# dkohlsdorf/audio_pattern_discovery

Hardware: AMD Instinct MI355X
Metric: DTW cell-updates/sec (whole node) (higher is better)
Workload: dtype f32

## Files before the change

audio_pattern_discovery_amd/csrc/apd_internal.h:

```cpp
#pragma once
#include <hip/hip_runtime.h>
#include <stdint.h>

#include <iterator>
#include <map>
#include <set>
#include <string>
#include <type_traits>
#include <utility>
#include <vector>

#include "../../include/apd.h"

struct apd_context;
namespace apd {

constexpr int kTile = 16;
constexpr int kSlotsPerTile = kTile * kTile;
constexpr int kWave = 64;

struct BandSpec {
    float pct;
    uint32_t explicit_band;
    int use_explicit;
    float ins, del, mat;
};

struct AlignLaunch {
    const float *d_frames;
    uint32_t frames_bytes;
    const uint32_t *d_seq_off;
    const float *d_seq_nmax;
    const uint4 *d_tiles;
    uint32_t n_tiles;
    uint32_t n_seq;
    uint32_t dim, dpad;
    BandSpec band;
    float *d_slab;
    const uint32_t *d_nonfinite;
    uint32_t w_max;
    uint32_t n_max;
    int variant;
    int hybrid;
    int strict;
    float tau;
};

constexpr int kKernelDims[] = {8, 10, 13, 16, 20, 26};
constexpr bool is_kernel_dim(uint32_t d) { for (int k : kKernelDims) if ((uint32_t)k == d) return true; return false; }
constexpr uint32_t kernel_dim(uint32_t d) { for (int k : kKernelDims) if ((uint32_t)k >= d) return (uint32_t)k; return d; }
constexpr int max_cells_per_lane(uint32_t d) { return d <= 13 ? 9 : (d <= 16 ? 7 : 5); }
constexpr int max_strip_columns(uint32_t d) { return d <= 10 ? 13 : (d <= 13 ? 11 : max_cells_per_lane(d)); }

struct KernelGeom {
    enum Family : uint8_t { Generic, Systolic, Wide, Strip, BandedStrip, SharedColumns };
    Family family = Generic;
    uint8_t lanes_or_waves = 0;
    uint8_t cells = 0;

    constexpr int encode() const
    {
        constexpr int base[] = {0, 0, 10000, 20000, 30000, 40000};
        return family == Generic ? 0 : base[family] + lanes_or_waves * 100 + cells;
    }
    static constexpr KernelGeom decode(int key)
    {
        const Family f = key >= 100 && key < 10000 ? Systolic : key >= 10000 && key < 20000 ? Wide
                       : key >= 20000 && key < 30000 ? Strip : key >= 30000 && key < 40000 ? BandedStrip
                       : key >= 40000 && key < 50000 ? SharedColumns : Generic;
        if (f == Generic) return KernelGeom{};
        return KernelGeom{f, (uint8_t)((key % 10000) / 100), (uint8_t)(key % 100)};
    }
    constexpr uint32_t lanes_per_pair() const
    {
        return family == Systolic || family == SharedColumns ? lanes_or_waves : family == Wide ? 64u * lanes_or_waves : 64u;
    }
    constexpr uint32_t capacity() const { return (family == Wide ? 64u : 1u) * lanes_or_waves * cells; }
    constexpr bool operator==(KernelGeom o) const { return family == o.family && lanes_or_waves == o.lanes_or_waves && cells == o.cells; }
    constexpr bool operator<(KernelGeom o) const { return encode() < o.encode(); }
};

#define APD_SYSTOLIC_GEOMS(X) X(8, 5) X(8, 7) X(8, 9) X(16, 2) X(16, 3) X(16, 5) X(16, 7) X(16, 9) X(32, 5) X(32, 7) X(32, 9) \
                              X(64, 3) X(64, 5) X(64, 7) X(64, 9)
#define APD_WIDE_GEOMS(X) X(2, 5) X(2, 7) X(2, 9) X(4, 5) X(4, 7) X(4, 9) X(8, 5) X(8, 7) X(8, 9)
#define APD_STRIP_GEOMS(X) X(1, 3) X(1, 5) X(1, 7) X(1, 9) X(1, 11) X(1, 13) X(2, 3) X(2, 5) X(2, 7) X(2, 9) X(2, 11) X(2, 13) \
                           X(4, 3) X(4, 5) X(4, 7) X(4, 9) X(4, 11) X(4, 13)
#define APD_BANDED_STRIP_GEOMS(X) X(1, 5) X(1, 9) X(4, 5) X(4, 9)
#define APD_SHARED_COLUMN_GEOMS(X) X(16, 9)

#define APD_SYSTOLIC_ENTRY_(A, B) KernelGeom{KernelGeom::Systolic, A, B},
#define APD_WIDE_ENTRY_(A, B) KernelGeom{KernelGeom::Wide, A, B},
#define APD_STRIP_ENTRY_(A, B) KernelGeom{KernelGeom::Strip, A, B},
#define APD_BANDED_STRIP_ENTRY_(A, B) KernelGeom{KernelGeom::BandedStrip, A, B},
#define APD_SHARED_COLUMN_ENTRY_(A, B) KernelGeom{KernelGeom::SharedColumns, A, B},
constexpr KernelGeom kSystolicGeoms[] = {APD_SYSTOLIC_GEOMS(APD_SYSTOLIC_ENTRY_)};
constexpr KernelGeom kWideGeoms[] = {APD_WIDE_GEOMS(APD_WIDE_ENTRY_)};
constexpr KernelGeom kStripGeoms[] = {APD_STRIP_GEOMS(APD_STRIP_ENTRY_)};
constexpr KernelGeom kBandedStripGeoms[] = {APD_BANDED_STRIP_GEOMS(APD_BANDED_STRIP_ENTRY_)};
constexpr KernelGeom kSharedColumnGeoms[] = {APD_SHARED_COLUMN_GEOMS(APD_SHARED_COLUMN_ENTRY_)};
#undef APD_SYSTOLIC_ENTRY_
#undef APD_WIDE_ENTRY_
#undef APD_STRIP_ENTRY_
#undef APD_BANDED_STRIP_ENTRY_
#undef APD_SHARED_COLUMN_ENTRY_

template <class F, size_t... I>
bool with_kernel_dim_(uint32_t dim, F &&f, std::index_sequence<I...>)
{
    return ((dim == (uint32_t)kKernelDims[I] ? (f(std::integral_constant<int, kKernelDims[I]>{}), true) : false) || ...);
}
template <class F>
bool with_kernel_dim(uint32_t dim, F &&f) { return with_kernel_dim_(dim, f, std::make_index_sequence<std::size(kKernelDims)>{}); }

constexpr bool geom_instantiated(KernelGeom g, uint32_t dim)
{
    if (g.family == KernelGeom::Generic) return true;
    if (!is_kernel_dim(dim)) return false;
    const bool strip = g.family == KernelGeom::Strip;
    if (g.cells > (strip ? max_strip_columns(dim) : max_cells_per_lane(dim))) return false;
    auto on = [g](const auto &list) { for (KernelGeom e : list) if (e == g) return true; return false; };
    return g.family == KernelGeom::Systolic ? on(kSystolicGeoms) : g.family == KernelGeom::Wide ? on(kWideGeoms)
         : g.family == KernelGeom::SharedColumns ? on(kSharedColumnGeoms) : strip ? on(kStripGeoms) : on(kBandedStripGeoms);
}
template <size_t N>
constexpr bool geoms_round_trip(const KernelGeom (&list)[N])
{
    for (KernelGeom g : list) if (!(KernelGeom::decode(g.encode()) == g)) return false;
    return true;
}
static_assert(geoms_round_trip(kSystolicGeoms) && geoms_round_trip(kWideGeoms) && geoms_round_trip(kStripGeoms) &&
                  geoms_round_trip(kBandedStripGeoms) && geoms_round_trip(kSharedColumnGeoms), "a listed geometry has no integer code of its own");

__host__ __device__ constexpr int sweep_result_offset(int rows, int cols, int w) { return (cols - 1) - (rows - 1) + w; }
__host__ __device__ constexpr int sweep_capture_step(int rows, int cols, int w, int c)
{
    return (rows - 1) + sweep_result_offset(rows, cols, w) / c;
}
__host__ __device__ constexpr int sweep_steps_needed(int rows, int cols, int w, int c) { return sweep_capture_step(rows, cols, w, c) + 1; }
static_assert(sweep_result_offset(1000, 1024, 66) == 90 && sweep_capture_step(1000, 1024, 66, 9) == 1009 &&
                  sweep_steps_needed(1000, 1024, 66, 9) == 1010, "cfg 3's shape, rows the shorter sequence: lane 10 ends the sweep");
static_assert(sweep_steps_needed(1024, 1000, 66, 9) == 1028, "the same pair with the longer sequence as rows: u* = 42, lane 4");
static_assert(sweep_capture_step(40, 72, 34, 9) == 39 + 7 && (2 * 34 + 1 + 8) / 9 == 8,
              "|n - m| = w - 2: u* = 2w - 2 sits in the last active lane, nothing is cut at the end");
static_assert(sweep_steps_needed(2, 2, 2, 2) == 3 && sweep_steps_needed(72, 40, 34, 9) == 72, "smallest pair; u* = 2: lane 0");

constexpr int shared_column_unroll(int c) { return (c + 1) % 2 == 0 ? c + 1 : 2 * (c + 1); }
constexpr int shared_column_ring_min(int g, int c) { return (g - 1) * (c - 1) + 1 + 2 * shared_column_unroll(c); }
constexpr int shared_column_ring_frames(int g, int c) { return (shared_column_ring_min(g, c) + 16 + 7) / 8 * 8; }
constexpr uint32_t shared_column_slack(KernelGeom g)
{
    return (uint32_t)(shared_column_ring_frames(g.lanes_or_waves, g.cells) - shared_column_ring_min(g.lanes_or_waves, g.cells));
}
inline uint32_t host_w(const BandSpec &b, uint32_t n, uint32_t m);
inline bool shared_columns_qualify(const std::vector<uint32_t> &lens, uint32_t tile_a, uint32_t tile_b, const BandSpec &band,
                                   uint32_t slack)
{
    const uint32_t n_seq = (uint32_t)lens.size();
    for (uint32_t sa = 0; sa < (uint32_t)kTile; sa += 4)
        for (uint32_t sb = 0; sb < (uint32_t)kTile; sb += 4) {
            uint32_t lo = 0xFFFFFFFFu, hi = 0;
            for (uint32_t i = 0; i < 16; ++i) {
                const uint32_t a = tile_a * kTile + sa + i / 4, b = tile_b * kTile + sb + i % 4;
                if (!(a < b && b < n_seq) || lens[a] < 2 || lens[b] < 2) continue;
                const uint32_t w = host_w(band, lens[a], lens[b]);
                lo = w < lo ? w : lo;
                hi = w > hi ? w : hi;
            }
            if (hi > lo && hi - lo > slack) return false;
        }
    return true;
}

constexpr uint64_t strip_lds_bytes(uint32_t dim, uint32_t ppw, bool banded, uint32_t rows)
{
    const uint64_t dp = (dim + 4) & ~3u;
    return 4 * ((ppw == 1 ? 128 : 64) * dp + (uint64_t)ppw * (banded ? 2 : 1) * (rows + 4) + 16);
}

constexpr uint32_t kPathMaxOffsets = 20480;
__host__ __device__ constexpr uint32_t path_cells_per_lane(uint32_t w) { return (2 * w + 1 + 63) / 64 < 2 ? 2u : (2 * w + 1 + 63) / 64; }
inline uint64_t path_dir_words(uint32_t n, uint32_t m, uint32_t w)
{
    if (n < 2 || m < 2) return 0;
    return ((uint64_t)n + 63) * ((path_cells_per_lane(w) + 15) / 16) * 64;
}
struct PathPair {
    uint32_t px, py;
    uint64_t dir_off;
    uint64_t step_off;
};
struct PathLaunch {
    const float *d_frames;
    const uint32_t *d_seq_off;
    uint32_t dim, dpad;
    BandSpec band;
    const PathPair *d_pairs;
    uint32_t n_pairs;
    uint32_t *d_dirs;
    apd_path_step *d_steps;
    uint32_t *d_len;
    float *d_scores;
};
hipError_t launch_path_sweep(const PathLaunch &L, uint32_t c_max, hipStream_t stream);
hipError_t launch_path_trace(const PathLaunch &L, hipStream_t stream);

hipError_t launch_align(const AlignLaunch &L, KernelGeom g, hipStream_t stream, std::string &err, int *status);
hipError_t launch_generic_fallback(const AlignLaunch &L, hipStream_t stream, bool *fits);
bool generic_fallback_fits(uint32_t w_max);

struct TileClass { KernelGeom geom; uint32_t first, count, w_max, n_max; };
void plan_tile_classes(const std::vector<uint64_t> &offsets, uint32_t n_seq, const std::vector<uint2> &tiles, const BandSpec &band,
                       uint32_t dim, int variant, bool fast_ok, bool uniform_pen, bool fast_shift, std::vector<TileClass> &classes,
                       std::vector<uint4> &flat);
hipError_t launch_pad(const float *d_src, float *d_dst, const uint32_t *d_seq_off, const uint32_t *d_src_off, uint32_t n_seq,
                      uint64_t n_frames_padded, uint32_t src_dim, uint32_t dim, uint32_t dpad, uint32_t *d_flags, float *d_seq_nmax,
                      hipStream_t stream);
hipError_t launch_unpack(const float *d_gathered, float *d_out, const uint32_t *d_order, uint32_t n_seq, uint32_t world,
                         uint64_t slab_floats, const uint32_t *d_flags, uint32_t *d_status, hipStream_t stream);
hipError_t launch_selftest(int *d_result, hipStream_t stream);
hipError_t launch_join_flags(uint32_t *d_flags_out, const uint32_t *d_flags_a, const uint32_t *d_flags_b, hipStream_t stream);
hipError_t launch_unpack_cross(const float *d_slab, float *d_fs, float *d_sf, const uint32_t *d_order, uint32_t n_seq, uint32_t n0,
                               uint32_t n_first, bool swapped, const uint32_t *d_flags, uint32_t *d_status, hipStream_t stream);
hipError_t launch_cross_linkage(const float *d_fs, const float *d_sf, uint32_t n_first, uint32_t n_second, const uint32_t *d_members,
                                const uint32_t *d_set_off, uint32_t n_sets, float *d_link, uint32_t *d_nearest, float *d_nearest_linkage,
                                hipStream_t stream);
hipError_t launch_sqrt_sweep(uint32_t first, uint64_t count, unsigned long long *d_out, hipStream_t stream);
constexpr float kFeatureFloor = 0x1p-40f;
constexpr float kFeatureBound = 0x1p60f;

struct DeviceBuf {
    void *ptr = nullptr;
    size_t bytes = 0;
    DeviceBuf() = default;
    DeviceBuf(DeviceBuf &&o) noexcept : ptr(o.ptr), bytes(o.bytes) { o.ptr = nullptr; o.bytes = 0; }
    DeviceBuf &operator=(DeviceBuf &&o) noexcept { std::swap(ptr, o.ptr); std::swap(bytes, o.bytes); return *this; }
    ~DeviceBuf() { reset(); }
    hipError_t reset() { const hipError_t e = ptr ? hipFree(ptr) : hipSuccess; ptr = nullptr; bytes = 0; return e; }
    hipError_t alloc(size_t n)
    {
        if (hipError_t e = reset(); e != hipSuccess) return e;
        if (hipError_t e = hipMalloc(&ptr, n); e != hipSuccess) { ptr = nullptr; return e; }
        bytes = n;
        return hipSuccess;
    }
    hipError_t reserve(size_t n) { return ptr && bytes >= n ? hipSuccess : alloc(n); }
    template <class T> T *as() const { return static_cast<T *>(ptr); }
    explicit operator bool() const { return ptr != nullptr; }
};

struct ContextChild {
    apd_context *ctx = nullptr;
    virtual void release_device() = 0;
    virtual ~ContextChild() = default;
};
int destroy_child(ContextChild *child);

int device_select(apd_context *ctx, const float *d_x, uint64_t len, uint64_t k, float *value);
uint64_t percentile_index(uint64_t len, float perc);

inline uint32_t host_band_from_pct(float pct, uint32_t len)
{
    float p = pct * (float)len;
    if (!(p > 0.0f)) return 0;
    if (p >= 4294967040.0f) return 0xFFFFFFFFu;
    return (uint32_t)p;
}
inline uint32_t host_w(const BandSpec &b, uint32_t n, uint32_t m)
{
    uint32_t mx = n > m ? n : m, gap = n > m ? n - m : m - n;
    uint32_t band = b.use_explicit ? b.explicit_band : host_band_from_pct(b.pct, mx);
    if (band > mx) band = mx;
    return (band > gap ? band : gap) + 2;
}

extern thread_local const apd_context *tl_bound_context;
bool affinity_debug();
hipError_t bind_device(const apd_context *ctx);
bool affinity_ok(const apd_context *ctx, const char *where);

}

#define APD_AFFINITY(ctx, where)                                                                   \
    do { if (apd::affinity_debug() && !apd::affinity_ok((ctx), (where))) return APD_ERR_HIP; } while (0)

#define HIP_TRY(ctx, call)                                                             \
    do {                                                                               \
        if (hipError_t e_ = (call); e_ != hipSuccess) {                                \
            (ctx)->last_error = std::string(#call) + ": " + hipGetErrorString(e_);     \
            return e_ == hipErrorOutOfMemory ? APD_ERR_OOM : APD_ERR_HIP;              \
        }                                                                              \
    } while (0)

struct apd_context {
    int device = 0;
    hipStream_t stream = nullptr;
    bool own_stream = false;
    bool timing = false;
    hipEvent_t ev0 = nullptr, ev1 = nullptr;
    static constexpr int kSideStreams = 4;
    hipStream_t side[kSideStreams] = {nullptr, nullptr, nullptr, nullptr};
    hipEvent_t side_done[kSideStreams] = {nullptr, nullptr, nullptr, nullptr};
    hipEvent_t fork = nullptr;
    std::set<apd::ContextChild *> children;
    std::set<void *> buffers;
    bool timed = false;
    int variant = 0;
    int distance_mode = 1;
    float tau = 1.0f / 64.0f;
    std::string last_error;
    apd::DeviceBuf ws_linkage;
    apd::DeviceBuf ws_slab;
    apd::DeviceBuf ws_misc;
    apd::DeviceBuf ws_gather;
    apd::DeviceBuf ws_path_dirs;
    apd::DeviceBuf ws_path_steps;
    uint32_t *d_status = nullptr;
    uint32_t drop_tiles = 0;
    apd_batch *pair_batch = nullptr;
    uint64_t pair_n = 0, pair_m = 0;
    uint32_t pair_dim = 0;
};

inline int reserve_ws(apd_context *ctx, apd::DeviceBuf &ws, size_t need)
{
    APD_AFFINITY(ctx, "workspace allocation");
    HIP_TRY(ctx, ws.reserve(need));
    return APD_OK;
}

struct apd_batch : apd::ContextChild {
    uint32_t n_seq = 0, dim = 0, dpad = 0;
    uint32_t src_dim = 0;
    uint64_t total_frames = 0;
    apd::DeviceBuf d_frames;
    uint32_t frames_bytes = 0;
    apd::DeviceBuf d_meta;
    std::vector<uint32_t> h_meta;
    uint32_t *d_seq_off = nullptr;
    uint32_t *d_src_off = nullptr;
    uint32_t *d_order = nullptr;
    uint32_t *d_flags = nullptr;
    float *d_seq_nmax = nullptr;
    mutable int nonfinite = -1;
    std::vector<uint32_t> order;
    std::vector<uint64_t> offsets;
    uint32_t min_len = 0, max_len = 0;
    bool joined = false, swapped = false;
    uint32_t first_len = 0, seg0 = 0;
    struct TilePlan { apd::DeviceBuf d_tiles; std::vector<apd::TileClass> classes; };
    mutable std::map<std::string, TilePlan> tile_cache;
    void release_device() override;
};
```

audio_pattern_discovery_amd/csrc/dtw_systolic.h:

```cpp
#pragma once
#include <type_traits>

#ifndef APD_ABLATE
#define APD_ABLATE 0
#endif

#include "dtw_common.h"

namespace apd {

typedef float apd_f32x4 __attribute__((ext_vector_type(4)));
constexpr uint32_t kNoFrame = 0xFFFFFF00u;

template <int D>
__device__ __forceinline__ void load_frame(float (&dst)[D], __amdgpu_buffer_rsrc_t rsrc, uint32_t byte_off)
{
    constexpr int DP4 = (D + 3) / 4;
#pragma unroll
    for (int q = 0; q < DP4; ++q) {
        const apd_f32x4 t = __builtin_bit_cast(apd_f32x4, __builtin_amdgcn_raw_buffer_load_b128(rsrc, byte_off + 16u * q, 0, 0));
        if (4 * q + 0 < D) dst[4 * q + 0] = t.x;
        if (4 * q + 1 < D) dst[4 * q + 1] = t.y;
        if (4 * q + 2 < D) dst[4 * q + 2] = t.z;
        if (4 * q + 3 < D) dst[4 * q + 3] = t.w;
    }
}

template <int D>
__device__ __forceinline__ void load_frame_dwords(float (&dst)[D], __amdgpu_buffer_rsrc_t rsrc, uint32_t byte_off)
{
#pragma unroll
    for (int k = 0; k < D; ++k)
        dst[k] = __builtin_bit_cast(float, __builtin_amdgcn_raw_buffer_load_b32(rsrc, byte_off + 4u * k, 0, 0));
}

template <int D, int DN>
__device__ __forceinline__ float frame_dist(const float (&x)[DN], const float (&y)[DN])
{
    float t = x[0] - y[0];
    float acc = t * t;
#pragma unroll
    for (int k = 1; k < D; ++k) {
        t = x[k] - y[k];
        acc = __builtin_fmaf(t, t, acc);
    }
    if (APD_ABLATE & 1) return acc;
    return __builtin_amdgcn_sqrtf(acc);
}

template <int D, int DN>
__device__ __forceinline__ float frame_sq_strict(const float (&x)[DN], const float (&y)[DN])
{
    float t = x[0] - y[0];
    float acc = t * t;
#pragma unroll
    for (int k = 1; k < D; ++k) {
        t = x[k] - y[k];
        const float sq = t * t;
        acc = acc + sq;
    }
    return acc;
}
template <int D, int DN>
__device__ __forceinline__ float frame_dist_strict(const float (&x)[DN], const float (&y)[DN])
{
    return __builtin_sqrtf(frame_sq_strict<D, DN>(x, y));
}

template <int D>
__device__ __forceinline__ float frame_sq_expanded_pre(const float (&xm)[D + 1], const float (&y)[D + 1])
{
    float acc = xm[D] + y[D];
#pragma unroll
    for (int k = 0; k < D; ++k) acc = __builtin_fmaf(xm[k], y[k], acc);
    return acc;
}
template <int D>
__device__ __forceinline__ void prescale_row_piece(apd_f32x4 &v, int piece)
{
    const bool np = piece == D / 4;
    v.x = (np && D % 4 == 0) ? v.x : -2.0f * v.x;
    v.y = (np && D % 4 == 1) ? v.y : -2.0f * v.y;
    v.z = (np && D % 4 == 2) ? v.z : -2.0f * v.z;
    v.w = (np && D % 4 == 3) ? v.w : -2.0f * v.w;
}
template <int D>
__device__ __forceinline__ float frame_sq_exact_pre(const float (&xm)[D + 1], const float (&y)[D + 1])
{
    float t = __builtin_fmaf(-0.5f, xm[0], -y[0]);
    float acc = t * t;
#pragma unroll
    for (int k = 1; k < D; ++k) {
        t = __builtin_fmaf(-0.5f, xm[k], -y[k]);
        acc = __builtin_fmaf(t, t, acc);
    }
    return acc;
}
template <int C, int G, bool UNIFORM_PEN>
__device__ __forceinline__ void dp_rows_step(float (&prev1)[C], float (&prev2)[C], const float (&d)[C], const bool (&g1)[C],
                                             const bool (&g2)[C], float del, float ins, float mat, int gl)
{
    float left1 = group_from_lower_wrap<G>(prev1[C - 1], APD_INF, gl);
    float left2 = group_from_lower_wrap<G>(prev2[C - 1], APD_INF, gl);
    float upr1 = APD_INF, upr2 = APD_INF;
#pragma unroll
    for (int c = 0; c < C; ++c) {
        if (APD_ABLATE & 2) { prev1[c] += d[c]; prev2[c] -= d[c]; continue; }
        const float up1 = (c < C - 1) ? prev1[(c + 1) % C] : upr1;
        const float up2 = (c < C - 1) ? prev2[(c + 1) % C] : upr2;
        const float r1 = select_node<UNIFORM_PEN>(left1, up1, prev1[c], d[c], del, ins, mat, (APD_ABLATE & 16) ? false : g1[c]);
        const float r2 = select_node<UNIFORM_PEN>(up2, left2, prev2[c], d[c], del, ins, mat, (APD_ABLATE & 16) ? false : g2[c]);
        prev1[c] = r1; prev2[c] = r2;
        left1 = r1; left2 = r2;
        if (c == 0) {
            upr1 = group_from_upper_wrap<G>(r1, APD_INF, gl);
            upr2 = group_from_upper_wrap<G>(r2, APD_INF, gl);
        }
    }
}
template <int C>
__device__ __forceinline__ void slow_phase_captures(float (&prev1)[C], float (&prev2)[C], float &res1, float &res2, int tau, int gl,
                                                    int tau_cap, int cw, int cstar)
{
    if (tau == gl) {
#pragma unroll
        for (int c = 0; c < C; ++c) if (c == cw) { prev1[c] = 0.0f; prev2[c] = 0.0f; }
    }
    if (tau == tau_cap) {
#pragma unroll
        for (int c = 0; c < C; ++c) if (c == cstar) { res1 = prev1[c]; res2 = prev2[c]; }
    }
}
template <int D, int C, int G, bool UNIFORM_PEN, bool HYBRID>
__global__ __launch_bounds__(256) void dtw_fused_systolic(const AlignLaunch L)
{
    static_assert(C >= 2 && (64 % G) == 0, "bad geometry");
    if (L.d_nonfinite != nullptr && *L.d_nonfinite != 0u) return;
    constexpr int DN = D + 1;
    constexpr int DP = (DN + 3) & ~3;
    constexpr int PPW = 64 / G;
    constexpr int WPT = kSlotsPerTile / (4 * PPW);
    const int lane = threadIdx.x & 63;
    const int gl = lane % G;
    const uint32_t xcd = blockIdx.x & 7u, q = blockIdx.x >> 3;
    const uint32_t tile = (q / WPT) * 8u + xcd;
    const uint32_t slot = ((q % WPT) * 4u + (threadIdx.x >> 6)) * PPW + lane / G;
    const PairInfo P = decode_pair_rows_b(L, tile, slot);
    const bool special = P.valid && (P.n == 1 || P.m == 1);
    const bool sweep = P.valid && !special;
    if (__ballot(sweep) == 0ull) {
        if (special && gl == 0) { const float s = (P.n == 1 && P.m == 1) ? 0.0f : APD_INF; store_pair(L, tile, P, s, s); }
        return;
    }
    const int n = sweep ? P.n : 1, m = sweep ? P.m : 1, w = sweep ? P.w : 2;
    const __amdgpu_buffer_rsrc_t rsrc = __builtin_amdgcn_make_buffer_rsrc((void *)L.d_frames, 0, L.frames_bytes, 0x00020000);
    const uint32_t a_off = (uint32_t)(P.A - L.d_frames) * 4u, b_off = (uint32_t)(P.B - L.d_frames) * 4u;
    constexpr uint32_t FB = DP * 4u;
    float ins = L.band.ins, del = L.band.del, mat = L.band.mat;
    float tau_thr = L.tau, nmax_b = P.nmax_b;
    asm volatile("" : "+v"(ins), "+v"(del), "+v"(mat), "+v"(tau_thr), "+v"(nmax_b));
    constexpr int R = (G == 64) ? 128 : 64;
    constexpr int LPF = DP / 4;
    constexpr int FPF = 64 / LPF;
    constexpr int RS = DP + 4;
    constexpr int U_ROWS = ((C + 1) % 2 == 0) ? (C + 1) : 2 * (C + 1);
    __shared__ float xring_all[4][(R + U_ROWS) * RS];
    float *const xring = xring_all[threadIdx.x >> 6];
    const int lead = __builtin_ctzll(__ballot(sweep));
    const uint32_t a_off_w = __builtin_amdgcn_readlane(a_off, lead);
    const int n_w = __builtin_amdgcn_readlane(n, lead);
    const int u0 = C * gl;
    const int two_w = 2 * w;

    bool g1[C], g2[C];
#pragma unroll
    for (int c = 0; c < C; ++c) {
        const int u = u0 + c;
        g1[c] = u >= two_w;
        g2[c] = (u == 0) | (u > two_w);
    }
    const int cw = w - u0;
    const int ustar = sweep_result_offset(n, m, w);
    const int cstar = ustar - u0;
    const int tau_cap = (n - 1) + gl;

    int w_bound = w;
    asm volatile("" : "+v"(w_bound));
    int my_total = sweep ? sweep_steps_needed(n, m, w_bound, C) : 0;
    int my_min = sweep ? (n - 1) : 0x7fffffff;
    int total = 0, min_rows = 0x7fffffff;
#pragma unroll
    for (int g = 0; g < PPW; ++g) {
        total = max(total, __builtin_amdgcn_readlane(my_total, g * G));
        min_rows = min(min_rows, __builtin_amdgcn_readlane(my_min, g * G));
    }
    constexpr int S = C + 1;
    constexpr int U = (S % 2 == 0) ? S : 2 * S;
    static_assert(U == U_ROWS, "ring copy sized for another unroll");
    constexpr bool MASKED_FETCH = HYBRID && (G == 32 || G == 8) && !(APD_ABLATE & 512);
    const int total_r = ((total + U - 1) / U) * U;
    int a_steps = G;
    if (UNIFORM_PEN && !HYBRID) {
        int w_max = 0;
#pragma unroll
        for (int g = 0; g < PPW; ++g) w_max = max(w_max, __builtin_amdgcn_readlane(w, g * G));
        a_steps = max(G, w_max + 1);
    }
    const int a_end = min(((a_steps + U - 1) / U) * U, total_r);
    const int b_end = min(max((min_rows / U) * U, a_end), total_r);

    float prev1[C], prev2[C];
#pragma unroll
    for (int c = 0; c < C; ++c) { prev1[c] = APD_INF; prev2[c] = APD_INF; }
    float res1 = 0.0f, res2 = 0.0f;

    float yf[S][DN];
#pragma unroll
    for (int c = 0; c < C; ++c) {
        const int j = u0 - gl + c - w;
        const int idx = (j >= 1) ? (min(j, m) - 1) : (HYBRID ? m : m + 1);
        load_frame<DN>(yf[c], rsrc, b_off + (uint32_t)idx * FB);
    }
#pragma unroll
    for (int k = 0; k < DN; ++k) yf[C][k] = 0.0f;
    if (HYBRID && !MASKED_FETCH && !(APD_ABLATE & 8)) {
        const int jt = 1 + (C - 1) * G - w;
        const uint32_t yo = b_off + (uint32_t)((jt >= 1) ? (min(jt, m) - 1) : m) * FB;
        load_frame<DN>(yf[C], rsrc, gl == G - 1 ? yo : kNoFrame);
    }
    constexpr int NFILL = (U + FPF - 1) / FPF;
    const int fill_f = lane / LPF, fill_q = lane % LPF;
    auto fill_load = [&](int first_row, apd_f32x4 (&regs)[NFILL]) __attribute__((always_inline)) {
#pragma unroll
        for (int f = 0; f < NFILL; ++f) {
            const int fi = f * FPF + fill_f;
            const bool act = (fill_f < FPF) & (fi < U);
            const uint32_t off = a_off_w + (uint32_t)(min(first_row + fi, n_w) - 1) * FB + 16u * fill_q;
            regs[f] = __builtin_bit_cast(apd_f32x4, __builtin_amdgcn_raw_buffer_load_b128(rsrc, act ? off : kNoFrame, 0, 0));
        }
    };
    auto fill_store = [&](int first_row, const apd_f32x4 (&regs)[NFILL]) __attribute__((always_inline)) {
#pragma unroll
        for (int f = 0; f < NFILL; ++f) {
            const int fi = f * FPF + fill_f;
            if ((fill_f < FPF) & (fi < U)) {
                apd_f32x4 v = regs[f];
                if (HYBRID) prescale_row_piece<D>(v, fill_q);
                const int slot = (first_row + fi) & (R - 1);
                *reinterpret_cast<apd_f32x4 *>(&xring[slot * RS + 4 * fill_q]) = v;
                if (slot < U) *reinterpret_cast<apd_f32x4 *>(&xring[(slot + R) * RS + 4 * fill_q]) = v;
            }
        }
    };
    for (int e = lane; e < G * DP; e += 64) {
        const int slot = (-(e / DP)) & (R - 1);
        const float v = HYBRID ? ((e % DP) == D ? APD_INF : 0.0f) : -APD_INF;
        xring[slot * RS + (e % DP)] = v;
        if (slot < U) xring[(slot + R) * RS + (e % DP)] = v;
    }
    {
        apd_f32x4 regs[NFILL];
        fill_load(1, regs);
        fill_store(1, regs);
    }
    asm volatile("" ::: "memory");
    auto read_row = [&](float (&dst)[DN], int row) __attribute__((always_inline)) {
        const float *p = &xring[(row & (R - 1)) * RS];
#pragma unroll
        for (int q = 0; q < LPF; ++q) {
            const apd_f32x4 t = *reinterpret_cast<const apd_f32x4 *>(p + 4 * q);
            if (4 * q + 0 < DN) dst[4 * q + 0] = t.x;
            if (4 * q + 1 < DN) dst[4 * q + 1] = t.y;
            if (4 * q + 2 < DN) dst[4 * q + 2] = t.z;
            if (4 * q + 3 < DN) dst[4 * q + 3] = t.w;
        }
    };
    auto read_row_at = [&](float (&dst)[DN], const float *p) __attribute__((always_inline)) {
#pragma unroll
        for (int q = 0; q < LPF; ++q) {
            const apd_f32x4 t = *reinterpret_cast<const apd_f32x4 *>(p + 4 * q);
            if (4 * q + 0 < DN) dst[4 * q + 0] = t.x;
            if (4 * q + 1 < DN) dst[4 * q + 1] = t.y;
            if (4 * q + 2 < DN) dst[4 * q + 2] = t.z;
            if (4 * q + 3 < DN) dst[4 * q + 3] = t.w;
        }
    };
    constexpr int NX = HYBRID ? 1 : 2;
    float xs[NX][DN];
    read_row(xs[0], 0 - gl);
#pragma unroll
    for (int k = 0; k < DN; ++k) xs[NX - 1][k] = (NX == 1) ? xs[0][k] : 0.0f;
    constexpr bool PIPE = (APD_ABLATE & 32) != 0;
    float dn[C];
#pragma unroll
    for (int c = 0; c < C; ++c) dn[c] = (PIPE && !HYBRID && c < C - 1) ? frame_dist_strict<D, DN>(xs[0], yf[c]) : 0.0f;

    auto advance_window = [&](int q) __attribute__((always_inline)) {
        const int r = q % S, e = (r + C) % S;
#pragma unroll
        for (int k = 0; k < (HYBRID ? DN : D); ++k) {
            if (APD_ABLATE & 4) { yf[e][k] = yf[(r + 1) % S][k] + yf[e][k]; continue; }
            yf[e][k] = MASKED_FETCH ? dpp_move<(G == 8) ? 0x101 : 0x130>(yf[(r + 1) % S][k], yf[e][k])
                                    : group_from_upper<G>(yf[(r + 1) % S][k], yf[e][k], gl);
        }
    };
    auto macro_steps = [&](int tau_begin, int tau_end, auto slow_tag) __attribute__((always_inline)) {
        constexpr bool SLOW = decltype(slow_tag)::value;
        uint32_t yo_cur = kNoFrame, yo_cap = kNoFrame, yo_step = 0u;
        if (!SLOW && gl == G - 1) {
            yo_cap = b_off + (uint32_t)(m - 1) * FB;
            yo_cur = min(b_off + (uint32_t)(tau_begin + ((HYBRID && !MASKED_FETCH) ? 1 : 0) + (C - 1) * G - w) * FB, yo_cap);
            yo_step = FB;
        }
        auto fetch_column = [&](float (&dst)[DN], int t) __attribute__((always_inline)) {
            if (APD_ABLATE & 8) return;
            if (SLOW) {
                const int jt = t + 1 + (C - 1) * G - w;
                const uint32_t yo = b_off + (uint32_t)((jt >= 1) ? (min(jt, m) - 1) : (HYBRID ? m : m + 1)) * FB;
                load_frame<DN>(dst, rsrc, gl == G - 1 ? yo : kNoFrame);
            } else {
                load_frame<DN>(dst, rsrc, yo_cur);
                yo_cur = min(yo_cur + yo_step, yo_cap);
            }
        };
        for (int tau0 = tau_begin; tau0 < tau_end; tau0 += U) {
            apd_f32x4 fill_regs[NFILL];
            fill_load(tau0 + U + 1, fill_regs);
            const float *const xrows = &xring[((tau0 + 1 - gl) & (R - 1)) * RS];
#pragma unroll
            for (int q = 0; q < U; ++q) {
                const int tau = tau0 + q;
                const int r = q % S;
                const int xa = HYBRID ? 0 : (q & 1), xb = HYBRID ? 0 : (xa ^ 1);
                const int e = (r + C) % S;
                if (!HYBRID) {
                    fetch_column(yf[e], tau);
                    read_row_at(xs[xb], xrows + q * RS);
                }
                float d[C];
                if (HYBRID) {
#pragma unroll
                    for (int c = 0; c < C; ++c) {
                        d[c] = frame_sq_expanded_pre<D>(xs[xa], yf[(r + c) % S]);
                    }
                    float dmin = d[0];
#pragma unroll
                    for (int c = 1; c + 1 < C; c += 2) dmin = __builtin_fminf(__builtin_fminf(dmin, d[c]), d[c + 1]);
                    if (C % 2 == 0) dmin = __builtin_fminf(dmin, d[C - 1]);
                    const bool any = (APD_ABLATE & 128) ? false : dmin < (xs[xa][D] + nmax_b) * tau_thr;
                    advance_window(q);
                    if (MASKED_FETCH) {
                        if (gl == G - 1) fetch_column(yf[e], tau);
                    }
                    if (__builtin_expect(__ballot(any) != 0ull, 0)) {
                        float nx = xs[xa][D];
                        asm volatile("" : "+v"(nx));
#pragma unroll
                        for (int c = 0; c < C; ++c) {
                            const float sc = nx + yf[(r + c) % S][D];
                            const float ex = frame_sq_exact_pre<D>(xs[xa], yf[(r + c) % S]);
                            d[c] = (d[c] < sc * tau_thr) ? ex : d[c];
                        }
                    }
                    if (!MASKED_FETCH) fetch_column(yf[r], tau + 1);
#pragma unroll
                    for (int c = 0; c < C; ++c) d[c] = (APD_ABLATE & 1) ? d[c] : __builtin_amdgcn_sqrtf(d[c]);
                    read_row_at(xs[0], xrows + q * RS);
                } else if (UNIFORM_PEN && !SLOW && !PIPE) {
                    float d2[C];
#pragma unroll
                    for (int c = 0; c < C; ++c) d2[c] = frame_sq_strict<D, DN>(xs[xa], yf[(r + c) % S]);
                    float dmin = d2[0];
#pragma unroll
                    for (int c = 1; c + 1 < C; c += 2) dmin = __builtin_fminf(__builtin_fminf(dmin, d2[c]), d2[c + 1]);
                    if (C % 2 == 0) dmin = __builtin_fminf(dmin, d2[C - 1]);
                    if (__builtin_expect(__ballot(!(dmin >= 0x1p-96f)) != 0ull, 0)) {
#pragma unroll
                        for (int c = 0; c < C; ++c) d[c] = __builtin_sqrtf(d2[c]);
                    } else {
#pragma unroll
                        for (int c = 0; c < C; ++c) d[c] = sqrt_rn_finite(d2[c]);
                    }
                } else {
#pragma unroll
                    for (int c = 0; c < C; ++c)
                        d[c] = (UNIFORM_PEN && PIPE && c < C - 1) ? dn[c] : frame_dist_strict<D, DN>(xs[xa], yf[(r + c) % S]);
                    if (PIPE) {
#pragma unroll
                        for (int c = 0; c < C - 1; ++c) dn[c] = frame_dist_strict<D, DN>(xs[xb], yf[(r + 1 + c) % S]);
                    }
                }
                dp_rows_step<C, G, UNIFORM_PEN>(prev1, prev2, d, g1, g2, del, ins, mat, gl);
                if (SLOW) slow_phase_captures<C>(prev1, prev2, res1, res2, tau, gl, tau_cap, cw, cstar);
                if (!HYBRID) advance_window(q);
            }
            fill_store(tau0 + U + 1, fill_regs);
            asm volatile("" ::: "memory");
        }
    };
    macro_steps(0, a_end, std::true_type{});
    macro_steps(a_end, b_end, std::false_type{});
    macro_steps(b_end, total_r, std::true_type{});

    if (P.valid && gl == (sweep ? ustar / C : 0)) {
        if (sweep) {
            const float denom = (float)(n + m);
            store_pair_rows_b(L, tile, P, res1 / denom, res2 / denom);
        } else {
            const float s = (P.n == 1 && P.m == 1) ? 0.0f : APD_INF;
            store_pair(L, tile, P, s, s);
        }
    }
}

typedef float apd_f32x2 __attribute__((ext_vector_type(2)));
template <int DN>
__device__ __forceinline__ void read_frame_lds(float (&dst)[DN], const float *p)
{
    constexpr int FULL = DN / 4, TAIL = DN % 4;
#pragma unroll
    for (int k = 0; k < FULL; ++k) {
        const apd_f32x4 t = *reinterpret_cast<const apd_f32x4 *>(p + 4 * k);
        dst[4 * k + 0] = t.x; dst[4 * k + 1] = t.y; dst[4 * k + 2] = t.z; dst[4 * k + 3] = t.w;
    }
    if (TAIL >= 2) {
        const apd_f32x2 t = *reinterpret_cast<const apd_f32x2 *>(p + 4 * FULL);
        dst[4 * FULL + 0] = t.x; dst[4 * FULL + 1] = t.y;
    }
    if (TAIL == 1) dst[4 * FULL] = p[4 * FULL];
    if (TAIL == 3) dst[4 * FULL + 2] = p[4 * FULL + 2];
}

constexpr int shared_column_ring_floats(int rc, int u, int dp) { return (((rc + u) * dp + ((rc + u + 7) / 8) * 4) * 4 + 255) / 256 * 64; }

template <int D, int C, int G>
__global__ __launch_bounds__(256) void dtw_fused_systolic_shared(const AlignLaunch L)
{
    static_assert(C >= 2 && G == 16, "one ring per wavefront: four lane groups");
    if (L.d_nonfinite != nullptr && *L.d_nonfinite != 0u) return;
    constexpr int DN = D + 1;
    constexpr int DP = (DN + 3) & ~3;
    constexpr int PPW = 64 / G;
    constexpr int WPT = kSlotsPerTile / (4 * PPW);
    constexpr int S = C + 1;
    constexpr int U = shared_column_unroll(C);
    constexpr int RC = shared_column_ring_frames(G, C);
    constexpr int R = 64;
    constexpr int LPF = DP / 4;
    constexpr int FPF = 64 / LPF;
    constexpr int RS = DP + 4;
    constexpr uint32_t FB = DP * 4u;
    constexpr int XRING = (R + U) * RS;
    constexpr int CRING = shared_column_ring_floats(RC, U, DP);
    static_assert(FPF >= U && RC % 8 == 0, "one wave-wide load per fill");
    static_assert(RC >= (G - 1) * (C - 1) + 2 * U + (int)shared_column_slack(KernelGeom{KernelGeom::SharedColumns, G, C}),
                  "ring too short for the spread of w the tile plan admits");
    extern __shared__ __attribute__((aligned(16))) float apd_shared_lds[];
    const int lane = threadIdx.x & 63, wave = threadIdx.x >> 6;
    const int gl = lane % G;
    float *const xring = apd_shared_lds + wave * XRING;
    float *const crings = apd_shared_lds + 4 * XRING;
    int *const wg_words = reinterpret_cast<int *>(crings + PPW * CRING);
    const uint32_t xcd = blockIdx.x & 7u, q = blockIdx.x >> 3;
    const uint32_t tile = (q / WPT) * 8u + xcd;
    const uint32_t sub = q % WPT;
    const uint32_t slot = ((sub % 4u) * 4u + wave) * kTile + (sub / 4u) * 4u + lane / G;
    const PairInfo P = decode_pair_rows_b(L, tile, slot);
    const bool special = P.valid && (P.n == 1 || P.m == 1);
    const bool sweep = P.valid && !special;
    const int n = sweep ? P.n : 1, m = sweep ? P.m : 1, w = sweep ? P.w : 2;
    const int u0 = C * gl;
    const int two_w = 2 * w;
    int w_bound = w;
    asm volatile("" : "+v"(w_bound));
    int my_total = sweep ? sweep_steps_needed(n, m, w_bound, C) : 0;
    int my_min = sweep ? (n - 1) : 0x7fffffff;
    int my_w = sweep ? w : 0x7fffffff;
    int total = 0, min_rows = 0x7fffffff, w_lo = 0x7fffffff;
#pragma unroll
    for (int g = 0; g < PPW; ++g) {
        total = max(total, __builtin_amdgcn_readlane(my_total, g * G));
        min_rows = min(min_rows, __builtin_amdgcn_readlane(my_min, g * G));
        w_lo = min(w_lo, __builtin_amdgcn_readlane(my_w, g * G));
    }
    if (lane == 0) { wg_words[2 * wave] = total; wg_words[2 * wave + 1] = w_lo; }
    __syncthreads();
    total = 0; w_lo = 0x7fffffff;
#pragma unroll
    for (int k = 0; k < 4; ++k) { total = max(total, wg_words[2 * k]); w_lo = min(w_lo, wg_words[2 * k + 1]); }
    if (total == 0) {
        if (special && gl == 0) { const float s = (P.n == 1 && P.m == 1) ? 0.0f : APD_INF; store_pair(L, tile, P, s, s); }
        return;
    }
    const __amdgpu_buffer_rsrc_t rsrc = __builtin_amdgcn_make_buffer_rsrc((void *)L.d_frames, 0, L.frames_bytes, 0x00020000);
    const uint32_t a_off = (uint32_t)(P.A - L.d_frames) * 4u, b_off = (uint32_t)(P.B - L.d_frames) * 4u;
    float ins = L.band.ins, del = L.band.del, mat = L.band.mat;
    float tau_thr = L.tau, nmax_b = P.nmax_b;
    asm volatile("" : "+v"(ins), "+v"(del), "+v"(mat), "+v"(tau_thr), "+v"(nmax_b));
    const unsigned long long sweeping = __ballot(sweep);
    const int lead = sweeping ? __builtin_ctzll(sweeping) : 0;
    const uint32_t a_off_w = sweeping ? __builtin_amdgcn_readlane(a_off, lead) : 0u;
    const int n_w = sweeping ? __builtin_amdgcn_readlane(n, lead) : 1;
    uint32_t cb_off = 0u;
    int cm = 0;
    bool cvalid = false;
    {
        const uint4 t = L.d_tiles[tile];
        const uint32_t a = t.x * kTile + (sub / 4u) * 4u + wave;
        if (a < L.n_seq) {
            const uint32_t oa = L.d_seq_off[a];
            cm = (int)(L.d_seq_off[a + 1] - oa) - 2;
            cb_off = oa * L.dpad * 4u;
            cvalid = true;
        }
    }

    bool g1[C], g2[C];
#pragma unroll
    for (int c = 0; c < C; ++c) {
        const int u = u0 + c;
        g1[c] = u >= two_w;
        g2[c] = (u == 0) | (u > two_w);
    }
    const int cw = w - u0;
    const int ustar = sweep_result_offset(n, m, w);
    const int cstar = ustar - u0;
    const int tau_cap = (n - 1) + gl;
    const int total_r = ((total + U - 1) / U) * U;
    const int a_end = min(((G + U - 1) / U) * U, total_r);
    const int b_end = min(max((min_rows / U) * U, a_end), total_r);

    float prev1[C], prev2[C];
#pragma unroll
    for (int c = 0; c < C; ++c) { prev1[c] = APD_INF; prev2[c] = APD_INF; }
    float res1 = 0.0f, res2 = 0.0f;

    float yf[S][DN];
#pragma unroll
    for (int c = 0; c < C; ++c) {
        const int j = u0 - gl + c - w;
        const int idx = (j >= 1) ? (min(j, m) - 1) : m;
        load_frame<DN>(yf[c], rsrc, b_off + (uint32_t)idx * FB);
    }
#pragma unroll
    for (int k = 0; k < DN; ++k) yf[C][k] = 0.0f;

    constexpr int NFILL = (U + FPF - 1) / FPF;
    const int fill_f = lane / LPF, fill_q = lane % LPF;
    const bool fill_act = (fill_f < FPF) & (fill_f < U);
    auto fill_load = [&](int first_row, apd_f32x4 (&regs)[NFILL]) __attribute__((always_inline)) {
        const uint32_t off = a_off_w + (uint32_t)(min(first_row + fill_f, n_w) - 1) * FB + 16u * fill_q;
        regs[0] = __builtin_bit_cast(apd_f32x4, __builtin_amdgcn_raw_buffer_load_b128(rsrc, fill_act ? off : kNoFrame, 0, 0));
    };
    auto fill_store = [&](int first_row, const apd_f32x4 (&regs)[NFILL]) __attribute__((always_inline)) {
        if (fill_act) {
            apd_f32x4 v = regs[0];
            prescale_row_piece<D>(v, fill_q);
            const int rslot = (first_row + fill_f) & (R - 1);
            *reinterpret_cast<apd_f32x4 *>(&xring[rslot * RS + 4 * fill_q]) = v;
            if (rslot < U) *reinterpret_cast<apd_f32x4 *>(&xring[(rslot + R) * RS + 4 * fill_q]) = v;
        }
    };
    for (int e = lane; e < G * DP; e += 64) {
        const int rslot = (-(e / DP)) & (R - 1);
        const float v = (e % DP) == D ? APD_INF : 0.0f;
        xring[rslot * RS + (e % DP)] = v;
        if (rslot < U) xring[(rslot + R) * RS + (e % DP)] = v;
    }
    {
        apd_f32x4 regs[NFILL];
        fill_load(1, regs);
        fill_store(1, regs);
    }
    float *const cring_fill = crings + wave * CRING;
    const int col_hi0 = U + (C - 1) * G - w_lo;
    auto ring_slot = [](int j) { return (j + 64 * RC) % RC; };
    auto ring_at = [](auto *ring, uint32_t p) { return ring + p * DP + ((p >> 3) << 2); };
    auto col_load = [&](int j, bool act) __attribute__((always_inline)) {
        const int idx = (j >= 1) ? (min(j, cm) - 1) : cm;
        const uint32_t off = cb_off + (uint32_t)idx * FB + 16u * fill_q;
        return __builtin_bit_cast(apd_f32x4, __builtin_amdgcn_raw_buffer_load_b128(rsrc, (act & cvalid) ? off : kNoFrame, 0, 0));
    };
    for (int j0 = col_hi0 - RC + 1; j0 <= col_hi0; j0 += FPF) {
        const int j = j0 + fill_f;
        const bool act = (fill_f < FPF) & (j <= col_hi0);
        const apd_f32x4 v = col_load(j, act);
        const uint32_t ps = (uint32_t)ring_slot(j);
        if (act) *reinterpret_cast<apd_f32x4 *>(ring_at(cring_fill, ps) + 4 * fill_q) = v;
        if (act && ps < (uint32_t)U) *reinterpret_cast<apd_f32x4 *>(ring_at(cring_fill, ps + RC) + 4 * fill_q) = v;
    }
    uint32_t pf = (uint32_t)ring_slot(col_hi0 + 1 + fill_f);
    const float *const cring_read = crings + (lane / G) * CRING;
    uint32_t pr = (uint32_t)ring_slot(1 + (C - 1) * (gl + 1) - w);
    auto read_col = [&](float (&dst)[DN], const float *block_base, int q) __attribute__((always_inline)) {
        read_frame_lds<DN>(dst, block_base + q * DP + (((pr + (uint32_t)q) >> 3) << 2));
    };
    __syncthreads();
    auto read_row_at = [&](float (&dst)[DN], const float *p) __attribute__((always_inline)) { read_frame_lds<DN>(dst, p); };
    float xs[DN];
    read_row_at(xs, &xring[((0 - gl) & (R - 1)) * RS]);

    auto macro_steps = [&](int tau_begin, int tau_end, auto slow_tag) __attribute__((always_inline)) {
        constexpr bool SLOW = decltype(slow_tag)::value;
        for (int tau0 = tau_begin; tau0 < tau_end; tau0 += U) {
            apd_f32x4 fill_regs[NFILL];
            fill_load(tau0 + U + 1, fill_regs);
            const apd_f32x4 col_regs = col_load(tau0 + col_hi0 + 1 + fill_f, fill_act);
            const float *const xrows = &xring[((tau0 + 1 - gl) & (R - 1)) * RS];
            const float *const ycols = cring_read + pr * DP;
#pragma unroll
            for (int q = 0; q < U; ++q) {
                const int tau = tau0 + q;
                const int r = q % S;
                const int e = (r + C) % S;
                float d[C];
#pragma unroll
                for (int c = 0; c < C; ++c) d[c] = frame_sq_expanded_pre<D>(xs, yf[(r + c) % S]);
                float dmin = d[0];
#pragma unroll
                for (int c = 1; c + 1 < C; c += 2) dmin = __builtin_fminf(__builtin_fminf(dmin, d[c]), d[c + 1]);
                if (C % 2 == 0) dmin = __builtin_fminf(dmin, d[C - 1]);
                const bool any = dmin < (xs[D] + nmax_b) * tau_thr;
                read_col(yf[e], ycols, q);
                if (__builtin_expect(__ballot(any) != 0ull, 0)) {
                    float nx = xs[D];
                    asm volatile("" : "+v"(nx));
#pragma unroll
                    for (int c = 0; c < C; ++c) {
                        const float sc = nx + yf[(r + c) % S][D];
                        const float ex = frame_sq_exact_pre<D>(xs, yf[(r + c) % S]);
                        d[c] = (d[c] < sc * tau_thr) ? ex : d[c];
                    }
                }
#pragma unroll
                for (int c = 0; c < C; ++c) d[c] = __builtin_amdgcn_sqrtf(d[c]);
                read_row_at(xs, xrows + q * RS);
                dp_rows_step<C, G, true>(prev1, prev2, d, g1, g2, del, ins, mat, gl);
                if (SLOW) slow_phase_captures<C>(prev1, prev2, res1, res2, tau, gl, tau_cap, cw, cstar);
            }
            fill_store(tau0 + U + 1, fill_regs);
            if (fill_act) *reinterpret_cast<apd_f32x4 *>(ring_at(cring_fill, pf) + 4 * fill_q) = col_regs;
            if (fill_act && pf < (uint32_t)U) *reinterpret_cast<apd_f32x4 *>(ring_at(cring_fill, pf + RC) + 4 * fill_q) = col_regs;
            pf = min(pf + (uint32_t)U, pf + (uint32_t)U - (uint32_t)RC);
            pr = min(pr + (uint32_t)U, pr + (uint32_t)U - (uint32_t)RC);
            __syncthreads();
        }
    };
    macro_steps(0, a_end, std::true_type{});
    macro_steps(a_end, b_end, std::false_type{});
    macro_steps(b_end, total_r, std::true_type{});

    if (P.valid && gl == (sweep ? ustar / C : 0)) {
        if (sweep) {
            const float denom = (float)(n + m);
            store_pair_rows_b(L, tile, P, res1 / denom, res2 / denom);
        } else {
            const float s = (P.n == 1 && P.m == 1) ? 0.0f : APD_INF;
            store_pair(L, tile, P, s, s);
        }
    }
}

template <int D, int C, int G>
constexpr size_t shared_columns_lds_bytes()
{
    constexpr int DP = (D + 1 + 3) & ~3, U = shared_column_unroll(C), RC = shared_column_ring_frames(G, C);
    constexpr int XRING = (64 + U) * (DP + 4), CRING = shared_column_ring_floats(RC, U, DP);
    return (size_t)(4 * XRING + (64 / G) * CRING + 8) * sizeof(float);
}
template <int D, int C, int G>
static hipError_t launch_shared_columns_kernel(const AlignLaunch &L, hipStream_t stream)
{
    constexpr int WPT = kSlotsPerTile / (4 * (64 / G));
    constexpr size_t lds = shared_columns_lds_bytes<D, C, G>();
    static_assert(lds <= 80 * 1024, "two workgroups per CU");
    static bool granted[64] = {};
    int dev = 0;
    if (hipError_t e = hipGetDevice(&dev); e != hipSuccess) return e;
    if (dev < 0 || dev >= 64 || !granted[dev]) {
        const hipError_t e = hipFuncSetAttribute(reinterpret_cast<const void *>(dtw_fused_systolic_shared<D, C, G>),
                                                 hipFuncAttributeMaxDynamicSharedMemorySize, (int)lds);
        if (e != hipSuccess) return e;
        if (dev >= 0 && dev < 64) granted[dev] = true;
    }
    const uint32_t tiles8 = (L.n_tiles + 7u) / 8u * 8u;
    hipLaunchKernelGGL((dtw_fused_systolic_shared<D, C, G>), dim3(tiles8 * WPT), dim3(256), lds, stream, L);
    return hipSuccess;
}

template <int D, int C, int G, bool UNIFORM_PEN, bool HYBRID>
static void launch_systolic_kernel(const AlignLaunch &L, hipStream_t stream)
{
    constexpr int PPW = 64 / G;
    constexpr int WPT = kSlotsPerTile / (4 * PPW);
    const uint32_t tiles8 = (L.n_tiles + 7u) / 8u * 8u;
    hipLaunchKernelGGL((dtw_fused_systolic<D, C, G, UNIFORM_PEN, HYBRID>), dim3(tiles8 * WPT), dim3(256), 0, stream, L);
}

#ifdef APD_SYSTOLIC_STRICT_UNIT
template <int D>
bool launch_systolic_strict(const AlignLaunch &L, KernelGeom g, hipStream_t stream)
{
#define APD_CASE(GG, CC) if constexpr (geom_instantiated(KernelGeom{KernelGeom::Systolic, GG, CC}, D)) { \
        if (g == KernelGeom{KernelGeom::Systolic, GG, CC}) { launch_systolic_kernel<D, CC, GG, true, false>(L, stream); return true; } }
    APD_SYSTOLIC_GEOMS(APD_CASE)
#undef APD_CASE
    return false;
}
#else
template <int D>
bool launch_systolic(const AlignLaunch &L, KernelGeom g, hipStream_t stream)
{
    const bool unit = L.band.ins == 1.0f && L.band.del == 1.0f && L.band.mat == 1.0f;
    if (g.family == KernelGeom::SharedColumns) {
        if (!(unit && L.hybrid)) return false;
#define APD_CASE(GG, CC) if constexpr (geom_instantiated(KernelGeom{KernelGeom::SharedColumns, GG, CC}, D)) { \
        if (g == KernelGeom{KernelGeom::SharedColumns, GG, CC}) return launch_shared_columns_kernel<D, CC, GG>(L, stream) == hipSuccess; }
        APD_SHARED_COLUMN_GEOMS(APD_CASE)
#undef APD_CASE
        return false;
    }
    if (unit && !L.hybrid) return launch_systolic_strict<D>(L, g, stream);
#define APD_CASE(GG, CC) if constexpr (geom_instantiated(KernelGeom{KernelGeom::Systolic, GG, CC}, D)) { \
        if (g == KernelGeom{KernelGeom::Systolic, GG, CC}) { \
            if (!unit) launch_systolic_kernel<D, CC, GG, false, false>(L, stream); else launch_systolic_kernel<D, CC, GG, true, true>(L, stream); \
            return true; } }
    APD_SYSTOLIC_GEOMS(APD_CASE)
#undef APD_CASE
    return false;
}
#endif

}
```

Baseline: 3219 billion.

## Skip leading dead sweep steps and trim the tail in shared-column DTW kernel

```diff
diff --git a/audio_pattern_discovery_amd/csrc/apd_internal.h b/audio_pattern_discovery_amd/csrc/apd_internal.h
--- a/audio_pattern_discovery_amd/csrc/apd_internal.h
+++ b/audio_pattern_discovery_amd/csrc/apd_internal.h
@@ -143,6 +143,9 @@
 static_assert(sweep_capture_step(40, 72, 34, 9) == 39 + 7 && (2 * 34 + 1 + 8) / 9 == 8,
               "|n - m| = w - 2: u* = 2w - 2 sits in the last active lane, nothing is cut at the end");
 static_assert(sweep_steps_needed(2, 2, 2, 2) == 3 && sweep_steps_needed(72, 40, 34, 9) == 72, "smallest pair; u* = 2: lane 0");
+__host__ __device__ constexpr int sweep_first_step(int w_min, int c) { return w_min / c; }
+static_assert(sweep_first_step(8, 9) == 0 && sweep_first_step(9, 9) == 1 && sweep_first_step(66, 9) == 7 && sweep_first_step(2, 9) == 0,
+              "w = 8: lane 0 injects at step 0; w = 9: lane 1 at step 1; cfg 3's w = 66: lane 7; the dummy pair's w = 2: no skip");
 
 constexpr int shared_column_unroll(int c) { return (c + 1) % 2 == 0 ? c + 1 : 2 * (c + 1); }
 constexpr int shared_column_ring_min(int g, int c) { return (g - 1) * (c - 1) + 1 + 2 * shared_column_unroll(c); }
diff --git a/audio_pattern_discovery_amd/csrc/dtw_systolic.h b/audio_pattern_discovery_amd/csrc/dtw_systolic.h
--- a/audio_pattern_discovery_amd/csrc/dtw_systolic.h
+++ b/audio_pattern_discovery_amd/csrc/dtw_systolic.h
@@ -525,10 +525,15 @@
     const int cw = w - u0;
     const int ustar = sweep_result_offset(n, m, w);
     const int cstar = ustar - u0;
-    const int tau_cap = (n - 1) + gl;
-    const int total_r = ((total + U - 1) / U) * U;
-    const int a_end = min(((G + U - 1) / U) * U, total_r);
-    const int b_end = min(max((min_rows / U) * U, a_end), total_r);
+    const int first = sweep_first_step(w_lo, C);
+    const int last0 = first + ((total - 1 - first) / U) * U;
+    const int inj_step = (sweep && cw >= 0 && cw < C) ? gl : -1;
+    const int cap_step = (sweep && cstar >= 0 && cstar < C) ? (n - 1) + gl : -1;
+    int inj_hi = -1;
+#pragma unroll
+    for (int g = 0; g < PPW; ++g) inj_hi = max(inj_hi, __builtin_amdgcn_readlane(sweep ? w_bound / C : -1, g * G));
+    const int a_end = min(inj_hi < 0 ? first : first + ((inj_hi - first) / U + 1) * U, last0);
+    const int b_end = min(max(first + (max(min_rows - first, 0) / U) * U, a_end), last0);
 
     float prev1[C], prev2[C];
 #pragma unroll
@@ -538,7 +543,7 @@
     float yf[S][DN];
 #pragma unroll
     for (int c = 0; c < C; ++c) {
-        const int j = u0 - gl + c - w;
+        const int j = first + u0 - gl + c - w;
         const int idx = (j >= 1) ? (min(j, m) - 1) : m;
         load_frame<DN>(yf[c], rsrc, b_off + (uint32_t)idx * FB);
     }
@@ -567,13 +572,19 @@
         xring[rslot * RS + (e % DP)] = v;
         if (rslot < U) xring[(rslot + R) * RS + (e % DP)] = v;
     }
+    for (int r0 = 1; r0 < first + 1; r0 += U) {
+        apd_f32x4 regs[NFILL];
+        fill_load(r0, regs);
+        fill_store(r0, regs);
+    }
     {
         apd_f32x4 regs[NFILL];
-        fill_load(1, regs);
-        fill_store(1, regs);
+        fill_load(first + 1, regs);
+        fill_store(first + 1, regs);
     }
     float *const cring_fill = crings + wave * CRING;
     const int col_hi0 = U + (C - 1) * G - w_lo;
+    const int col_hi1 = first + col_hi0;
     auto ring_slot = [](int j) { return (j + 64 * RC) % RC; };
     auto ring_at = [](auto *ring, uint32_t p) { return ring + p * DP + ((p >> 3) << 2); };
     auto col_load = [&](int j, bool act) __attribute__((always_inline)) {
@@ -581,24 +592,24 @@
         const uint32_t off = cb_off + (uint32_t)idx * FB + 16u * fill_q;
         return __builtin_bit_cast(apd_f32x4, __builtin_amdgcn_raw_buffer_load_b128(rsrc, (act & cvalid) ? off : kNoFrame, 0, 0));
     };
-    for (int j0 = col_hi0 - RC + 1; j0 <= col_hi0; j0 += FPF) {
+    for (int j0 = col_hi1 - RC + 1; j0 <= col_hi1; j0 += FPF) {
         const int j = j0 + fill_f;
-        const bool act = (fill_f < FPF) & (j <= col_hi0);
+        const bool act = (fill_f < FPF) & (j <= col_hi1);
         const apd_f32x4 v = col_load(j, act);
         const uint32_t ps = (uint32_t)ring_slot(j);
         if (act) *reinterpret_cast<apd_f32x4 *>(ring_at(cring_fill, ps) + 4 * fill_q) = v;
         if (act && ps < (uint32_t)U) *reinterpret_cast<apd_f32x4 *>(ring_at(cring_fill, ps + RC) + 4 * fill_q) = v;
     }
-    uint32_t pf = (uint32_t)ring_slot(col_hi0 + 1 + fill_f);
+    uint32_t pf = (uint32_t)ring_slot(col_hi1 + 1 + fill_f);
     const float *const cring_read = crings + (lane / G) * CRING;
-    uint32_t pr = (uint32_t)ring_slot(1 + (C - 1) * (gl + 1) - w);
+    uint32_t pr = (uint32_t)ring_slot(first + 1 + (C - 1) * (gl + 1) - w);
     auto read_col = [&](float (&dst)[DN], const float *block_base, int q) __attribute__((always_inline)) {
         read_frame_lds<DN>(dst, block_base + q * DP + (((pr + (uint32_t)q) >> 3) << 2));
     };
     __syncthreads();
     auto read_row_at = [&](float (&dst)[DN], const float *p) __attribute__((always_inline)) { read_frame_lds<DN>(dst, p); };
     float xs[DN];
-    read_row_at(xs, &xring[((0 - gl) & (R - 1)) * RS]);
+    read_row_at(xs, &xring[((first - gl) & (R - 1)) * RS]);
 
     auto macro_steps = [&](int tau_begin, int tau_end, auto slow_tag) __attribute__((always_inline)) {
         constexpr bool SLOW = decltype(slow_tag)::value;
@@ -613,6 +624,7 @@
                 const int tau = tau0 + q;
                 const int r = q % S;
                 const int e = (r + C) % S;
+                if (SLOW && q > 0 && tau >= total) return;
                 float d[C];
 #pragma unroll
                 for (int c = 0; c < C; ++c) d[c] = frame_sq_expanded_pre<D>(xs, yf[(r + c) % S]);
@@ -636,7 +648,16 @@
                 for (int c = 0; c < C; ++c) d[c] = __builtin_amdgcn_sqrtf(d[c]);
                 read_row_at(xs, xrows + q * RS);
                 dp_rows_step<C, G, true>(prev1, prev2, d, g1, g2, del, ins, mat, gl);
-                if (SLOW) slow_phase_captures<C>(prev1, prev2, res1, res2, tau, gl, tau_cap, cw, cstar);
+                if (SLOW) {
+                    const bool inj_now = tau == inj_step, cap_now = tau == cap_step;
+                    if (__ballot(inj_now | cap_now) != 0ull) {
+#pragma unroll
+                        for (int c = 0; c < C; ++c) {
+                            if (inj_now && c == cw) { prev1[c] = 0.0f; prev2[c] = 0.0f; }
+                            if (cap_now && c == cstar) { res1 = prev1[c]; res2 = prev2[c]; }
+                        }
+                    }
+                }
             }
             fill_store(tau0 + U + 1, fill_regs);
             if (fill_act) *reinterpret_cast<apd_f32x4 *>(ring_at(cring_fill, pf) + 4 * fill_q) = col_regs;
@@ -646,9 +667,9 @@
             __syncthreads();
         }
     };
-    macro_steps(0, a_end, std::true_type{});
+    macro_steps(first, a_end, std::true_type{});
     macro_steps(a_end, b_end, std::false_type{});
-    macro_steps(b_end, total_r, std::true_type{});
+    macro_steps(b_end, total, std::true_type{});
 
     if (P.valid && gl == (sweep ? ustar / C : 0)) {
         if (sweep) {
```

Measured after the change: 3249 billion, median of 6. Within noise of the previous version (+0.9%).
